# kianmcevoy/audio_analysis

Hardware: AMD Instinct MI355X
Metric: IRs/sec full report (STFT+RT60bands+zplane), 48 kHz 10 s IR (higher is better)
Workload: dtype f64; 1 GPU; metrics-only full report on 256 mono synthetic IRs per GPU per step, 10 s @ 48 kHz (SURVEY.md 8d generator), H2D included: every step uploads its batch from pinned host memory (float32, 492 MB) on a copy stream under the previous step's kernels; 4 distinct batches rotate; batch_per_gpu=256, parallelism=file-sharded dp1, gather=final

## Files before the change

### audio_analysis_amd/_lib.py

```python
from __future__ import annotations

import ctypes as C
from pathlib import Path

_LIB_PATH = Path(__file__).resolve().parent / "csrc" / "libira.so"
_lib = None
ABI_VERSION = 15

c_f32p = C.c_void_p
c_i64p = C.c_void_p
c_i32p = C.c_void_p
c_f64p = C.c_void_p
vp = C.c_void_p
i32 = C.c_int32
f64 = C.c_double
f32 = C.c_float

PROTOTYPES = {
    "ira_abi_version": (i32, []),
    "ira_error_string": (C.c_char_p, [i32]),
    "ira_peak_index": (i32, [vp, vp, vp, i32, C.c_int64, vp, vp, vp]),
    "ira_edc_db": (i32, [vp, vp, vp, i32, C.c_int64, f64, f64, vp, vp, vp, vp, vp]),
    "ira_curve_fits": (i32, [vp, vp, vp, i32, i32, f32, f32, vp, C.POINTER(f64), i32, i32, C.POINTER(f64), i32, i32,
                             f64, f64, vp, vp, vp]),
    "ira_edc_box_smooth": (i32, [vp, vp, vp, i32, C.c_int64, i32, f64, vp, vp]),
    "ira_edc_fits": (i32, [vp, vp, vp, i32, C.c_int64, f64, f64, f32, f32, C.POINTER(f64), i32, i32, C.POINTER(f64), i32,
                           vp, vp, vp, vp, vp, vp, vp, vp, vp, vp]),
    "ira_stft_mag_db": (i32, [vp, vp, vp, i32, i32, i32, i32, vp, vp, i32, f64, vp, vp, vp, vp, vp]),
    "ira_stft_logbin": (i32, [vp, vp, vp, i32, i32, i32, i32, vp, vp, i32, f64, i32, vp, vp, i32, vp, vp, vp]),
    "ira_stft_mag_db_tf": (i32, [vp, vp, vp, i32, i32, i32, i32, vp, vp, i32, f64, vp, vp, vp, vp, vp]),
    "ira_tail_energy": (i32, [vp, vp, vp, vp, i32, i32, vp, vp]),
    "ira_stft_logbin_tail": (i32, [vp, vp, vp, i32, i32, i32, i32, vp, vp, i32, f64, i32, vp, vp, i32, vp, vp, vp, vp, vp,
                                   vp]),
    "ira_stft_mag_db_tf_tail": (i32, [vp, vp, vp, i32, i32, i32, i32, vp, vp, i32, f64, vp, vp, vp, vp, vp, vp, vp, vp]),
    "ira_fft_split": (i32, [i32, vp, vp]),
    "ira_bluestein_filter": (i32, [vp, i32, i32, vp, vp, vp, vp, vp]),
    "ira_rfft_any": (i32, [vp, vp, vp, i32, i32, i32, vp, vp, vp, vp, vp, vp, vp, vp, vp, vp, vp, vp, i32, vp, vp, vp, vp,
                           vp, i32, vp]),
    "ira_band_irfft": (i32, [vp, vp, vp, i32, vp, vp, i32, vp, vp, vp, vp, vp, vp, vp, vp, vp, vp, vp]),
    "ira_spectrum_mag_phase": (i32, [vp, vp, vp, i32, i32, f64, vp, vp, vp, vp, vp, vp]),
    "ira_phase_unwrap": (i32, [vp, vp, vp, i32, i32, i32, vp, vp, vp, vp]),
    "ira_log_smooth_db": (i32, [vp, vp, vp, vp, vp, vp, vp, vp, vp, i32, i32, i32, i32, vp]),
    "ira_group_delay": (i32, [vp, vp, vp, i32, i32, vp, f64, vp, i32, vp, vp]),
    "ira_fft_smooth_split": (i32, [i32, vp, vp]),
    "ira_rfft_smooth": (i32, [vp, vp, i32, i32, i32, vp, vp, vp, vp, vp, vp, vp, vp, vp, vp, vp, vp, vp, vp, i32, vp]),
    "ira_band_irfft_smooth": (i32, [vp, vp, i32, i32, vp, vp, vp, vp, vp, vp, vp, vp, vp, vp, i32, vp, vp, vp]),
    "ira_band_tile_layout": (i32, [i32, i32, C.POINTER(i32), C.POINTER(i32)]),
    "ira_wav_probe": (i32, [C.c_char_p, vp, vp, vp, vp]),
    "ira_wav_read_pcm16": (i32, [C.c_char_p, C.c_int64, C.c_int64, i32, vp]),
    "ira_wav_probe_batch": (i32, [vp, i32, i32, vp, vp, vp, vp, vp]),
    "ira_wav_read_pcm16_batch": (i32, [vp, vp, vp, vp, vp, vp, i32, i32, vp]),
    "ira_pcm16_to_channels": (i32, [vp, C.c_int64, i32, i32, vp, vp]),
    "ira_pcm16_to_channels_jobs": (i32, [vp, vp, vp, vp, vp, vp, i32, C.c_int64, vp, vp]),
    "ira_band_mask_values": (i32, [C.POINTER(f64), f64, C.c_int64, vp, vp]),
    "ira_host_pull": (i32, [vp, C.c_int64, i32, vp, i32, vp]),
    "ira_deconv_divide": (i32, [vp, vp, vp, vp, vp, i32, i32, f64, vp, vp]),
    "ira_deconv_finish": (i32, [vp, vp, vp, vp, i32, i32, i32, i32, i32, f64, vp, vp, vp]),
    "ira_order_stats": (i32, [vp, vp, vp, i32, vp, i32, vp, vp]),
    "ira_diffusion": (i32, [vp, vp, vp, i32, i32, i32, i32, i32, f64, f64, vp, vp, vp, vp]),
    "ira_diffusion_stereo": (i32, [vp, vp, vp, vp, i32, i32, i32, i32, i32, vp, vp, vp, vp]),
    "ira_spectrum_stats": (i32, [vp, vp, vp, i32, vp, f64, f64, f64, vp, vp]),
    "ira_spectrum_finish": (i32, [vp, vp, vp, i32, f64, vp, vp, vp, i32, i32, vp, vp, vp, vp, f64, f64, f64, vp, vp]),
    "ira_waterfall_rel": (i32, [vp, vp, vp, i32, i32, i32, i32, f64, vp, vp, vp]),
    "ira_logbin_aggregate": (i32, [vp, vp, vp, i32, i32, i32, vp, vp, i32, vp, vp, i32, vp]),
    "ira_ar_partial_doubles": (C.c_int64, [i32, i32]),
    "ira_ar_gram": (i32, [vp, vp, vp, vp, vp, i32, i32, i32, vp, i32, vp]),
    "ira_ar_solve": (i32, [vp, vp, i32, i32, i32, f64, vp, vp, vp, i32, vp]),
# ... 87 lines not shown
```

### audio_analysis_amd/build.py

```python
from __future__ import annotations

import os
import shutil
import subprocess
import sys
from concurrent.futures import ThreadPoolExecutor
from pathlib import Path

CSRC = Path(__file__).resolve().parent / "csrc"
LIB = CSRC / "libira.so"
ARCH = "gfx950"

SOURCES = {
    "ira_api.hip": [],
    "ira_edc.hip": ["-ffp-contract=off"],
    "ira_stft.hip": ["-fno-slp-vectorize"],
    "ira_stft2.hip": ["-fno-slp-vectorize"],
    "ira_stft3.hip": ["-fno-slp-vectorize"],
    "ira_stft4.hip": [],
    "ira_tailenergy.hip": [],
    "ira_fftlong.hip": [],
    "ira_fftsmooth.hip": [],
    "ira_spectrum.hip": ["-ffp-contract=off"],
    "ira_modal.hip": ["-ffp-contract=off"],
    "ira_ar.hip": [],
    "ira_roots.hip": [],
    "ira_ingest.hip": ["-ffp-contract=off"],
    "ira_deconv.hip": ["-ffp-contract=off"],
    "ira_diffusion.hip": ["-ffp-contract=off"],
    "ira_energy.hip": ["-ffp-contract=off"],
    "ira_xcorr.hip": ["-ffp-contract=off"],
    "ira_lundeby.hip": ["-ffp-contract=off"],
    "ira_multislope.hip": ["-ffp-contract=off"],
    "ira_mtf.hip": [],
    "ira_harmonics.hip": ["-ffp-contract=off"],
    "ira_echo.hip": ["-ffp-contract=off"],
    "ira_echodensity.hip": ["-ffp-contract=off"],
    "ira_reflections.hip": ["-ffp-contract=off"],
    "ira_xspec.hip": [],
}
COMMON = ["-O3", "-std=c++17", "-fPIC", f"--offload-arch={ARCH}", "-Wall", "-Wno-unused-function"]


def _hipcc() -> str:
    exe = shutil.which("hipcc") or "/opt/rocm/bin/hipcc"
    if not Path(exe).exists():
        raise RuntimeError("hipcc not found; libira cannot be built")
    return exe


def _stale(obj: Path, deps) -> bool:
    if not obj.exists():
        return True
# ... 63 lines not shown
```

### audio_analysis_amd/csrc/ira_stft.h

```cpp
#pragma once
#include "ira_common.h"

int32_t ira_stft3_launch(const float* x, const int64_t* off, const int32_t* nframes, int32_t nseg, int32_t max_frames,
                         int32_t hop, const void* window, const void* tw, double floor_db, float* out,
                         const int64_t* out_off, const int32_t* frame_sel, const int64_t* sel_off, hipStream_t st);

int32_t ira_stft6_launch(const float* x, const int64_t* off, const int32_t* nframes, int32_t nseg, int32_t max_frames,
                         int32_t hop, const void* window, const void* tw, double floor_db, float* out,
                         const int64_t* out_off, const int32_t* frame_sel, const int64_t* sel_off, const double* tail,
                         const int64_t* tail_off, hipStream_t st);

int32_t ira_stft2_launch(const float* x, const int64_t* off, const int32_t* nframes, int32_t nseg, int32_t max_frames,
                         int32_t n_fft, int32_t hop, const void* window, const void* tw, int32_t precision,
                         double floor_db, float* out, const int64_t* out_off, const int32_t* frame_sel,
                         const int64_t* sel_off, hipStream_t st);

int32_t ira_stft5_launch(const float* x, const int64_t* off, const int32_t* nframes, int32_t nseg, int32_t max_frames,
                         int32_t hop, const void* window, const void* tw, double floor_db, float* out,
                         const int64_t* out_off, const int32_t* frame_sel, const int64_t* sel_off, int32_t lb_nbins,
                         int32_t lb_kbase, const int32_t* lb_first, const int32_t* lb_count, const double* tail,
                         const int64_t* tail_off, void* consts, hipStream_t st);
```

### audio_analysis_amd/csrc/ira_stft.hip

```cpp
#include <cmath>
#include <cstdlib>

#include "ira_fft_lds.h"
#include "ira_stft.h"

namespace {

using ira::cplx;

constexpr int STFT_THREADS = 256;

template <typename T>
__device__ __forceinline__ float mag_to_db(T re, T im, T floor_lin);

template <>
__device__ __forceinline__ float mag_to_db<float>(float re, float im, float floor_lin) {
  const float a = sqrtf(re * re + im * im);
  const float m = (a != a) ? a : fmaxf(a, floor_lin);
  return 20.0f * log10f(m);
}
template <>
__device__ __forceinline__ float mag_to_db<double>(double re, double im, double floor_lin) {
  const double a = hypot(re, im);
  const double m = (a != a) ? a : fmax(a, floor_lin);
// ... 91 lines not shown
                                   int32_t nseg, int32_t max_frames, int32_t n_fft, int32_t hop,
                                   const void* window_dev, const void* twiddle_dev, int32_t precision,
                                   double floor_db, float* out_dev, const int64_t* out_off_dev,
                                   const int32_t* frame_sel_dev, const int64_t* sel_off_dev, void* stream) {
  IRA_CHECK_PTR(x_dev); IRA_CHECK_PTR(off_dev); IRA_CHECK_PTR(nframes_dev); IRA_CHECK_PTR(window_dev);
  IRA_CHECK_PTR(twiddle_dev); IRA_CHECK_PTR(out_dev); IRA_CHECK_PTR(out_off_dev);
  if (frame_sel_dev != nullptr && sel_off_dev == nullptr) return IRA_E_NULL;
  if (nseg < 0 || max_frames < 0 || hop <= 0) return IRA_E_SIZE;
  if (nseg == 0 || max_frames == 0) return IRA_OK;
  if (n_fft < 64 || n_fft > 16384 || (n_fft & (n_fft - 1)) != 0) return IRA_E_SIZE;
  int log2n = 0;
  while ((1 << log2n) < n_fft) ++log2n;
  hipStream_t st = (hipStream_t)stream;
  if (precision != 32 && precision != 64) return IRA_E_UNSUPPORTED;
  if (precision == 32 && n_fft == 4096)
    return ira_stft3_launch(x_dev, off_dev, nframes_dev, nseg, max_frames, hop, window_dev, twiddle_dev, floor_db,
                            out_dev, out_off_dev, frame_sel_dev, sel_off_dev, st);
  if (n_fft == 8192 || (precision == 64 && n_fft == 4096))
    return ira_stft2_launch(x_dev, off_dev, nframes_dev, nseg, max_frames, n_fft, hop, window_dev, twiddle_dev,
                            precision, floor_db, out_dev, out_off_dev, frame_sel_dev, sel_off_dev, st);
  if (precision == 32)
    return launch_stft<float>(x_dev, off_dev, nframes_dev, nseg, max_frames, log2n, hop, window_dev, twiddle_dev,
                              floor_db, out_dev, out_off_dev, frame_sel_dev, sel_off_dev, st);
  return launch_stft<double>(x_dev, off_dev, nframes_dev, nseg, max_frames, log2n, hop, window_dev, twiddle_dev,
                             floor_db, out_dev, out_off_dev, frame_sel_dev, sel_off_dev, st);
}

namespace {

int32_t stft_mag_db_tf(const float* x_dev, const int64_t* off_dev, const int32_t* nframes_dev, int32_t nseg,
                       int32_t max_frames, int32_t n_fft, int32_t hop, const void* window_dev, const void* twiddle_dev,
                       int32_t precision, double floor_db, float* out_dev, const int64_t* out_off_dev,
                       const int32_t* frame_sel_dev, const int64_t* sel_off_dev, const double* tail_dev,
                       const int64_t* tail_off_dev, void* consts_dev, void* stream) {
  IRA_CHECK_PTR(x_dev); IRA_CHECK_PTR(off_dev); IRA_CHECK_PTR(nframes_dev); IRA_CHECK_PTR(window_dev);
  IRA_CHECK_PTR(twiddle_dev); IRA_CHECK_PTR(out_dev); IRA_CHECK_PTR(out_off_dev);
  if (frame_sel_dev != nullptr && sel_off_dev == nullptr) return IRA_E_NULL;
  if (nseg < 0 || max_frames < 0 || hop <= 0) return IRA_E_SIZE;
  if (nseg == 0 || max_frames == 0) return IRA_OK;
  if (nseg > 65535) return IRA_E_SIZE;
  hipStream_t st = (hipStream_t)stream;
  if (precision == 32 && n_fft == 4096)
    return ira_stft6_launch(x_dev, off_dev, nframes_dev, nseg, max_frames, hop, window_dev, twiddle_dev, floor_db,
                            out_dev, out_off_dev, frame_sel_dev, sel_off_dev, tail_dev, tail_off_dev, st);
  if (precision == 64 && n_fft == 8192)
    return ira_stft5_launch(x_dev, off_dev, nframes_dev, nseg, max_frames, hop, window_dev, twiddle_dev, floor_db,
                            out_dev, out_off_dev, frame_sel_dev, sel_off_dev, 0, 0, nullptr, nullptr, tail_dev,
                            tail_off_dev, consts_dev, st);
  return IRA_E_UNSUPPORTED;
}

int32_t stft_logbin(const float* x_dev, const int64_t* off_dev, const int32_t* nframes_dev, int32_t nseg,
                    int32_t max_frames, int32_t n_fft, int32_t hop, const void* window_dev, const void* twiddle_dev,
                    int32_t precision, double floor_db, int32_t k_base, const int32_t* first_dev,
                    const int32_t* count_dev, int32_t nbins, float* curves_dev, const int64_t* curves_off_dev,
                    const double* tail_dev, const int64_t* tail_off_dev, void* consts_dev, void* stream) {
  IRA_CHECK_PTR(x_dev); IRA_CHECK_PTR(off_dev); IRA_CHECK_PTR(nframes_dev); IRA_CHECK_PTR(window_dev);
  IRA_CHECK_PTR(twiddle_dev); IRA_CHECK_PTR(first_dev); IRA_CHECK_PTR(count_dev); IRA_CHECK_PTR(curves_dev);
  IRA_CHECK_PTR(curves_off_dev);
  if (nseg < 0 || max_frames < 0 || hop <= 0 || nbins <= 0 || k_base < 0) return IRA_E_SIZE;
  if (nseg == 0 || max_frames == 0) return IRA_OK;
  if (nseg > 65535) return IRA_E_SIZE;
  if (precision != 64 || n_fft != 8192) return IRA_E_UNSUPPORTED;
  return ira_stft5_launch(x_dev, off_dev, nframes_dev, nseg, max_frames, hop, window_dev, twiddle_dev, floor_db,
                          curves_dev, curves_off_dev, nullptr, nullptr, nbins, k_base, first_dev, count_dev, tail_dev,
                          tail_off_dev, consts_dev, (hipStream_t)stream);
}

}

extern "C" int32_t ira_stft_mag_db_tf(const float* x_dev, const int64_t* off_dev, const int32_t* nframes_dev,
                                      int32_t nseg, int32_t max_frames, int32_t n_fft, int32_t hop,
                                      const void* window_dev, const void* twiddle_dev, int32_t precision,
                                      double floor_db, float* out_dev, const int64_t* out_off_dev,
                                      const int32_t* frame_sel_dev, const int64_t* sel_off_dev, void* stream) {
  return stft_mag_db_tf(x_dev, off_dev, nframes_dev, nseg, max_frames, n_fft, hop, window_dev, twiddle_dev, precision,
                        floor_db, out_dev, out_off_dev, frame_sel_dev, sel_off_dev, nullptr, nullptr, nullptr, stream);
}

extern "C" int32_t ira_stft_mag_db_tf_tail(const float* x_dev, const int64_t* off_dev, const int32_t* nframes_dev,
                                           int32_t nseg, int32_t max_frames, int32_t n_fft, int32_t hop,
                                           const void* window_dev, const void* twiddle_dev, int32_t precision,
                                           double floor_db, float* out_dev, const int64_t* out_off_dev,
                                           const int32_t* frame_sel_dev, const int64_t* sel_off_dev,
                                           const double* tail_dev, const int64_t* tail_off_dev, void* consts_dev,
                                           void* stream) {
  return stft_mag_db_tf(x_dev, off_dev, nframes_dev, nseg, max_frames, n_fft, hop, window_dev, twiddle_dev, precision,
                        floor_db, out_dev, out_off_dev, frame_sel_dev, sel_off_dev, tail_dev, tail_off_dev, consts_dev,
                        stream);
}

extern "C" int32_t ira_stft_logbin(const float* x_dev, const int64_t* off_dev, const int32_t* nframes_dev,
                                   int32_t nseg, int32_t max_frames, int32_t n_fft, int32_t hop,
                                   const void* window_dev, const void* twiddle_dev, int32_t precision, double floor_db,
                                   int32_t k_base, const int32_t* first_dev, const int32_t* count_dev, int32_t nbins,
                                   float* curves_dev, const int64_t* curves_off_dev, void* stream) {
  return stft_logbin(x_dev, off_dev, nframes_dev, nseg, max_frames, n_fft, hop, window_dev, twiddle_dev, precision,
                     floor_db, k_base, first_dev, count_dev, nbins, curves_dev, curves_off_dev, nullptr, nullptr, nullptr,
                     stream);
}

extern "C" int32_t ira_stft_logbin_tail(const float* x_dev, const int64_t* off_dev, const int32_t* nframes_dev,
                                        int32_t nseg, int32_t max_frames, int32_t n_fft, int32_t hop,
                                        const void* window_dev, const void* twiddle_dev, int32_t precision,
                                        double floor_db, int32_t k_base, const int32_t* first_dev,
                                        const int32_t* count_dev, int32_t nbins, float* curves_dev,
                                        const int64_t* curves_off_dev, const double* tail_dev,
                                        const int64_t* tail_off_dev, void* consts_dev, void* stream) {
  return stft_logbin(x_dev, off_dev, nframes_dev, nseg, max_frames, n_fft, hop, window_dev, twiddle_dev, precision,
                     floor_db, k_base, first_dev, count_dev, nbins, curves_dev, curves_off_dev, tail_dev, tail_off_dev,
                     consts_dev, stream);
}
```

### audio_analysis_amd/csrc/ira_stft4.hip

```cpp
#include <cmath>
#include <cstdlib>

#include "ira_fft_reg.h"
#include "ira_log.h"
#include "ira_stft.h"

namespace {

using ira::brev_bits;
using ira::cplx;
using ira::dft_dif;
using ira::powers16;

typedef cplx<double> cdd;

constexpr int M4 = 4096, F4 = M4 + 1, TL4 = 128;
constexpr int ROW4 = 129;
constexpr int E2N4 = 256;
constexpr int EXC4 = 16 * ROW4;
static_assert(EXC4 >= 8 * E2N4 && EXC4 * 2 >= M4, "exchange buffer too small");

__device__ __forceinline__ float db_of4(double re, double im, double floor_pow, float floor_db,
                                        const ira::LogTabEntry* tab) {
  const double p = fma(re, re, im * im);
// ... 56 lines not shown
  for (int o = 32; o > 0; o >>= 1) {
    const unsigned long long other = __shfl_xor(wb, o, 64);
    wb = other > wb ? other : wb;
  }
  if ((q & 63) == 0) wmax[q >> 6] = wb;
  __syncthreads();
  unsigned long long wm = wmax[0];
#pragma unroll
  for (int i = 1; i < TL5 / 64; ++i) wm = wmax[i] > wm ? wmax[i] : wm;
  return ira::uniform(__longlong_as_double((long long)wm));
}

__global__ __launch_bounds__(TL5) void stft5_consts_kernel(const double* __restrict__ window, float floor_db, int lb_nbins,
                                                           const int32_t* __restrict__ lb_count, Stft5Consts* __restrict__ cst) {
  __shared__ unsigned long long wmax[TL5 / 64];
  __shared__ ira::LogTabEntry ltab[ira::LOGTAB_N];
  const int q = threadIdx.x;
  ira::build_log_table(ltab, q);
  const double wmax2 = window_max_sq5(window, q, wmax);
  if (q == 0) cst->wmax2 = wmax2;
  const double floor_lin32 = ira::uniform(exp10((double)floor_db * 0.05));
  for (int bb = q; bb < lb_nbins; bb += TL5) {
    const int c = lb_count[bb];
    cst->row[bb] = c > 0 ? logbin_mean_db<true>(nullptr, floor_lin32, c, ltab) : __uint_as_float(0x7fc00000u);
  }
}

__global__ __launch_bounds__(TL5) __attribute__((amdgpu_waves_per_eu(4, 4))) void stft5_kernel(
    const float* __restrict__ x, const int64_t* __restrict__ off, const int32_t* __restrict__ nframes, int hop,
    const double* __restrict__ window, const cdd* __restrict__ tw, double floor_lin, float floor_db,
    float* __restrict__ out, const int64_t* __restrict__ out_off, const int32_t* __restrict__ frame_sel,
    const int64_t* __restrict__ sel_off, int lb_nbins, int lb_kbase, const int32_t* __restrict__ lb_first,
    const int32_t* __restrict__ lb_count, int kfr, int ablate, const double* __restrict__ tail,
    const int64_t* __restrict__ tail_off, const Stft5Consts* __restrict__ cst) {
  __shared__ __attribute__((aligned(16))) cdd ex[EXC4];
  __shared__ double wave_energy[2][TL5 / 64];
  __shared__ double chunk_energy[TL5 / 64];
  __shared__ unsigned long long chunk_wmax[TL5 / 64];
  __shared__ float quiet_val[TL5];
  __shared__ ira::LogTabEntry ltab[ira::LOGTAB_N];
  __shared__ int lb_range[2];
  __shared__ int frame_bad;
  unsigned bx, by;
  ira::xcd_remap(bx, by);
  const int seg = (int)by;
  const int col0 = (int)bx * kfr;
  const int T_out = ira::uniform(nframes[seg]);
  if (col0 >= T_out) return;
  const int col1 = T_out - col0 < kfr ? T_out : col0 + kfr;
  int q = threadIdx.x;
  float* os = out + ira::uniform(out_off[seg]);
  const double floor_pow = floor_lin * floor_lin;

  const bool use_tail = tail != nullptr && frame_sel == nullptr && !IRA_ABL(ablate & (256 | 512));
  if (use_tail) {
    const int64_t j = ((int64_t)col0 * hop) / IRA_TAIL_BLOCK;
    const double S = ira::uniform(tail[ira::uniform(tail_off[seg]) + j]);
    const double wmax2 = ira::uniform(cst->wmax2);
    if (S * (4.0 * (2 * M4)) * wmax2 <= floor_pow) {
      const int nfr = col1 - col0;
      if (lb_nbins <= 0) {
        float* fo = os + (int64_t)col0 * F4;
        for (int i = q; i < nfr * F4; i += TL5) fo[i] = floor_db;
      } else {
        for (int bb = q; bb < lb_nbins; bb += TL5) {
          const float val = cst->row[bb];
          float* o = os + (int64_t)bb * T_out + col0;
          for (int jf = 0; jf < nfr; ++jf) o[jf] = val;
        }
      }
      return;
    }
  }

  double* exd = reinterpret_cast<double*>(ex);
  ira::build_log_table(ltab, q);
  if (q < 2) lb_range[q] = q == 0 ? F4 : 0;

  const float* xs = x + ira::uniform(off[seg]);
// ... 237 lines not shown
        if (!need_a && !need_b) continue;
        const cdd e = {0.5 * (zkr[i] + zpr[i]), 0.5 * (zki[i] - zpi[i])};
        const cdd d = {0.5 * (zkr[i] - zpr[i]), 0.5 * (zki[i] + zpi[i])};
        const cdd o = {d.im, -d.re};
        const cdd wk = ira::cmul(wlane, wuni[i]);
        const cdd pp = ira::cmul(wk, o);
        if (IRA_ABL(ablate & 4)) {
          if (need_a) exd[k] = e.re + pp.re;
          if (need_b) exd[M4 - k] = e.im - pp.im;
          continue;
        }
        if (need_a) exd[k] = lin_of4(e.re + pp.re, e.im + pp.im, floor_pow, floor_db, floor_lin32, ltab);
        if (need_b) exd[M4 - k] = lin_of4(e.re - pp.re, e.im - pp.im, floor_pow, floor_db, floor_lin32, ltab);
      }
      if (q == 0 && M4 / 2 >= k_lo && M4 / 2 < k_hi) exd[M4 / 2] = lin_of4(midr, midi, floor_pow, floor_db, floor_lin32, ltab);
    }
    __syncthreads();
    for (int bb = q; bb < lb_nbins; bb += TL5) {
      const int c = lb_count[bb];
      float val = qnan32;
      if (c > 0) val = logbin_mean_db<false>(exd + lb_kbase + lb_first[bb], 0.0, c, ltab);
      os[(int64_t)bb * T_out + col] = (bad_frame && c > 0) ? qnan32 : val;
    }
    __syncthreads();
  }
}

}

int32_t ira_stft5_launch(const float* x, const int64_t* off, const int32_t* nframes, int32_t nseg, int32_t max_frames,
                         int32_t hop, const void* window, const void* tw, double floor_db, float* out,
                         const int64_t* out_off, const int32_t* frame_sel, const int64_t* sel_off, int32_t lb_nbins,
                         int32_t lb_kbase, const int32_t* lb_first, const int32_t* lb_count, const double* tail,
                         const int64_t* tail_off, void* consts, hipStream_t st) {
  const double floor_lin = std::pow(10.0, floor_db / 20.0);
  int kfr = ira_tune_int("IRA_STFT5_K", KF5);
  if (kfr < 1) kfr = 1;
  if (frame_sel != nullptr) tail = nullptr;
  if (tail != nullptr) {
    if (tail_off == nullptr || consts == nullptr) return IRA_E_NULL;
    stft5_consts_kernel<<<1, TL5, 0, st>>>(static_cast<const double*>(window), (float)floor_db, lb_nbins > 0 ? lb_nbins : 0,
                                           lb_count, static_cast<Stft5Consts*>(consts));
    IRA_TRY_HIP(hipGetLastError());
  }
  dim3 grid((max_frames + kfr - 1) / kfr, nseg);
  stft5_kernel<<<grid, TL5, (size_t)ira_tune_int("IRA_STFT5_LDS_PAD", 0), st>>>(x, off, nframes, hop, static_cast<const double*>(window),
                                     static_cast<const cdd*>(tw), floor_lin, (float)floor_db, out, out_off, frame_sel,
                                     sel_off, lb_nbins, lb_kbase, lb_first, lb_count, kfr, ira_tune_int("IRA_STFT5_ABLATE", 0),
                                     tail, tail_off, static_cast<const Stft5Consts*>(consts));
  IRA_RETURN_LAUNCH();
}
```

### audio_analysis_amd/engine.py

```python
from __future__ import annotations

import ctypes
import math
import os
from contextlib import contextmanager
from dataclasses import dataclass, fields
from typing import Dict, List, Optional, Sequence, Tuple

import numpy as np

from . import _lib
from ._lib import IraError, check
from .engine_plan import (SMOOTH, Switches, conv_size, exclusive_cumsum, pair_bands, plan_band_irfft,
                          plan_rfft)

FIT_DOUBLES = 8
EDC_SCRATCH_DOUBLES = 4096
EDC_TILE = 4096


def _ptr(t) -> int:
    return 0 if t is None else int(t.data_ptr())


# ... 980 lines not shown
        if not np.array_equal(np.asarray(tail["start"]), np.asarray(seg_off, dtype=np.int64)):
            raise ValueError("the suffix-energy table was made for other segment starts")
        last = np.asarray(seg_off, dtype=np.int64) + (cols.astype(np.int64) - 1) * int(hop) + int(n_fft)
        if np.any((cols > 0) & (last > np.asarray(tail["end"]))):
            raise ValueError("a frame reads past the end the suffix-energy table was made for")
        return tail["tab"], tail["off_dev"]

    def stft_mag_db(self, x_dev, seg_off: np.ndarray, nframes: np.ndarray, n_fft: int, hop: int, use_hann: bool,
                    floor_db: float, precision: int = 32, frame_sel: Optional[List[np.ndarray]] = None,
                    frame_major: bool = False, tail=None):
        t = self.torch
        n = int(seg_off.size)
        f = n_fft // 2 + 1
        if self.stft_generic_needed(n_fft):
            return self._stft_generic(x_dev, seg_off, nframes, int(n_fft), int(hop), use_hann, floor_db, frame_sel,
                                      frame_major)
        if frame_sel is not None:
            cols = np.array([int(s.size) for s in frame_sel], dtype=np.int32)
            sel_off = exclusive_cumsum(cols)
            if cols.sum():
                sel, sel_off_dev = self.job_tables(np.concatenate(frame_sel).astype(np.int32), sel_off)
            else:
                sel, sel_off_dev = self.empty(1, t.int32), self.to_dev(sel_off)
        else:
            cols = np.ascontiguousarray(nframes, dtype=np.int32)
            sel = None
            sel_off_dev = None
        sizes = cols.astype(np.int64) * f
        out_off = exclusive_cumsum(sizes)
        out = self.empty(int(sizes.sum()), t.float32)
        d_off, d_cols, d_ooff = self.job_tables(seg_off, cols, out_off)
        use_tail = tail is not None and frame_major and frame_sel is None and self.stft_tail_ok(n_fft, precision) and n > 0
        name = "ira_stft_mag_db_tf_tail" if use_tail else "ira_stft_mag_db_tf" if frame_major else "ira_stft_mag_db"
        extra = ()
        if use_tail:
            d_tab, d_toff = self._tail_args(tail, seg_off, cols, n_fft, hop)
            consts = self.empty(1, t.float64)
            extra = (_ptr(d_tab), _ptr(d_toff), _ptr(consts))
        with self.tagged(f"[f{precision},n{n_fft}{',sel' if frame_sel is not None else ''}]"):
            check(getattr(self.lib, name)(
                _ptr(x_dev), _ptr(d_off), _ptr(d_cols), n, int(cols.max()) if n else 0, int(n_fft), int(hop),
                _ptr(self.window(n_fft, use_hann, precision)), _ptr(self.twiddle(n_fft, precision)), int(precision),
                float(floor_db), _ptr(out), _ptr(d_ooff), _ptr(sel), _ptr(sel_off_dev), *extra, self.stream), name)
        return out, out_off, cols

    def stft_logbin(self, x_dev, seg_off: np.ndarray, nframes: np.ndarray, n_fft: int, hop: int, use_hann: bool,
                    floor_db: float, k_base: int, first: np.ndarray, count: np.ndarray, tail=None):
        t = self.torch
        n = int(seg_off.size)
        nbins = int(first.size)
        cols = np.ascontiguousarray(nframes, dtype=np.int32)
        sizes = cols.astype(np.int64) * nbins
        out_off = exclusive_cumsum(sizes)
        out = self.empty(int(sizes.sum()), t.float32)
        d_off, d_cols, d_ooff, d_f, d_c = self.job_tables(seg_off, cols, out_off, first.astype(np.int32),
                                                           count.astype(np.int32))
        name, extra = "ira_stft_logbin", ()
        if tail is not None and n > 0:
            d_tab, d_toff = self._tail_args(tail, seg_off, cols, n_fft, hop)
            name = "ira_stft_logbin_tail"
            consts = self.empty(1 + (nbins + 1) // 2, t.float64)
            extra = (_ptr(d_tab), _ptr(d_toff), _ptr(consts))
        with self.tagged(f"[f64,n{n_fft}]"):
            check(getattr(self.lib, name)(_ptr(x_dev), _ptr(d_off), _ptr(d_cols), n, int(cols.max()) if n else 0,
                                          int(n_fft), int(hop), _ptr(self.window(n_fft, use_hann, 64)),
                                          _ptr(self.twiddle(n_fft, 64)), 64, float(floor_db), int(k_base), _ptr(d_f),
                                          _ptr(d_c), nbins, _ptr(out), _ptr(d_ooff), *extra, self.stream), name)
        return out, out_off

    @staticmethod
    def stft_generic_needed(n_fft: int) -> bool:
        n = int(n_fft)
        return n < 64 or n > 16384 or (n & (n - 1)) != 0

    def _stft_generic(self, x_dev, seg_off, nframes, n_fft: int, hop: int, use_hann: bool, floor_db: float, frame_sel,
                      frame_major: bool):
        t = self.torch
        n = int(seg_off.size)
        f = n_fft // 2 + 1
        if frame_sel is not None:
            frames = [np.asarray(s_, dtype=np.int64) for s_ in frame_sel]
        else:
            frames = [np.arange(int(c), dtype=np.int64) for c in nframes]
        cols = np.array([fr.size for fr in frames], dtype=np.int32)
        sizes = cols.astype(np.int64) * f
        out_off = exclusive_cumsum(sizes)
        total_frames = int(cols.sum())
        if total_frames == 0:
            return self.empty(1, t.float32), out_off, cols
        xoff = np.concatenate([int(seg_off[i]) + fr * int(hop) for i, fr in enumerate(frames)])
        lengths = np.full(total_frames, n_fft, dtype=np.int32)
        spec, spec_off = self.rfft_any(x_dev, xoff, lengths, bool(use_hann))
        mag, _ = self.spectrum_mag_phase(spec, spec_off, lengths, float(floor_db), want_phase=False)
        if frame_major:
            return mag, out_off, cols
# ... 502 lines not shown
```

### include/ira.h

```cpp
#ifndef IRA_H_
#define IRA_H_

#include <stdint.h>

#ifdef __cplusplus
extern "C" {
#endif

#define IRA_OK 0
#define IRA_E_NULL (-1)
#define IRA_E_SIZE (-2)
#define IRA_E_UNSUPPORTED (-3)
#define IRA_E_IO (-4)
#define IRA_E_FORMAT (-5)
#define IRA_E_HIP_BASE (-1000)

#define IRA_ABI_VERSION 15

int32_t ira_abi_version(void);
const char* ira_error_string(int32_t code);

int32_t ira_peak_index(const float* x_dev, const int64_t* off_dev, const int64_t* len_dev,
                       int32_t nseg, int64_t max_len, int64_t* peak_dev, float* peak_abs_dev, void* stream);

// ... 27 lines not shown
                        const void* window_dev, const void* twiddle_dev, int32_t precision,
                        double floor_db, float* out_dev, const int64_t* out_off_dev,
                        const int32_t* frame_sel_dev, const int64_t* sel_off_dev, void* stream);

int32_t ira_stft_mag_db_tf(const float* x_dev, const int64_t* off_dev, const int32_t* nframes_dev,
                           int32_t nseg, int32_t max_frames, int32_t n_fft, int32_t hop,
                           const void* window_dev, const void* twiddle_dev, int32_t precision,
                           double floor_db, float* out_dev, const int64_t* out_off_dev,
                           const int32_t* frame_sel_dev, const int64_t* sel_off_dev, void* stream);

int32_t ira_stft_logbin(const float* x_dev, const int64_t* off_dev, const int32_t* nframes_dev, int32_t nseg,
                        int32_t max_frames, int32_t n_fft, int32_t hop, const void* window_dev,
                        const void* twiddle_dev, int32_t precision, double floor_db, int32_t k_base,
                        const int32_t* first_dev, const int32_t* count_dev, int32_t nbins, float* curves_dev,
                        const int64_t* curves_off_dev, void* stream);

#define IRA_TAIL_BLOCK 512
int32_t ira_tail_energy(const float* x_dev, const int64_t* start_dev, const int64_t* end_dev,
                        const int64_t* tab_off_dev, int32_t nseg, int32_t max_nblk, double* tab_dev, void* stream);

#define IRA_STFT_CONSTS_DOUBLES(nbins) (1 + ((nbins) + 1) / 2)
int32_t ira_stft_logbin_tail(const float* x_dev, const int64_t* off_dev, const int32_t* nframes_dev, int32_t nseg,
                             int32_t max_frames, int32_t n_fft, int32_t hop, const void* window_dev,
                             const void* twiddle_dev, int32_t precision, double floor_db, int32_t k_base,
                             const int32_t* first_dev, const int32_t* count_dev, int32_t nbins, float* curves_dev,
                             const int64_t* curves_off_dev, const double* tail_dev, const int64_t* tail_off_dev,
                             void* consts_dev, void* stream);
int32_t ira_stft_mag_db_tf_tail(const float* x_dev, const int64_t* off_dev, const int32_t* nframes_dev,
                                int32_t nseg, int32_t max_frames, int32_t n_fft, int32_t hop,
                                const void* window_dev, const void* twiddle_dev, int32_t precision,
                                double floor_db, float* out_dev, const int64_t* out_off_dev,
                                const int32_t* frame_sel_dev, const int64_t* sel_off_dev, const double* tail_dev,
                                const int64_t* tail_off_dev, void* consts_dev, void* stream);


int32_t ira_fft_split(int32_t m, int32_t* n1, int32_t* n2);

int32_t ira_bluestein_filter(const int32_t* L_dev, int32_t nfilt, int32_t m, const void* t1_dev,
                             const void* t2_dev, const void* tf_dev, double* bfilt_dev, void* stream);

int32_t ira_rfft_any(const float* x_dev, const int64_t* xoff_dev, const int32_t* L_dev, int32_t nb,
                     int32_t use_hann, int32_t m, const void* t1_dev, const void* t2_dev,
                     const void* tf_dev, const double* bfilt_dev, const int32_t* bidx_dev,
                     double* work_dev, double* spec_out_dev, const int64_t* spec_off_dev,
                     const int64_t* x2off_dev, const int64_t* spec_off2_dev, double* zpair_dev,
                     const int64_t* zpair_off_dev, int32_t max_len, const int32_t* data_len_dev,
                     const int32_t* win_len_dev, const int32_t* data_len2_dev, const int32_t* win_len2_dev,
                     const int32_t* interleave_dev, int32_t keep_packed, void* stream);

#define IRA_BAND_DOUBLES 8
int32_t ira_band_irfft(const double* spec_dev, const int64_t* spec_off_dev, const int32_t* L_dev,
                       int32_t nb, const double* band_params_dev, const double* freq_val_dev,
                       int32_t m, const void* t1_dev, const void* t2_dev, const void* tf_dev,
                       const double* bfilt_dev, const int32_t* bidx_dev, double* work_dev, float* y_dev,
                       const int64_t* y1_off_dev, const int64_t* y2_off_dev,
                       const int64_t* spec_off2_dev, void* stream);

int32_t ira_spectrum_mag_phase(const double* spec_dev, const int64_t* spec_off_dev, const int32_t* L_dev,
                               int32_t nb, int32_t max_len, double floor_db, float* mag_db_dev,
                               const int64_t* mag_off_dev, double* phase_dev,
                               const int64_t* phase_off_dev, const int32_t* packed_dev, void* stream);

int32_t ira_phase_unwrap(const double* phase_dev, const int64_t* phase_off_dev, const int32_t* L_dev,
                         int32_t nb, int32_t do_unwrap, int32_t to_degrees, float* out_dev,
                         const int64_t* out_off_dev, double* out64_dev, void* stream);

// ... 247 lines not shown
```

Baseline: 17580 IRs/s.

## Cut STFT frames below the noise floor using tail-energy bounds and compact grid

Adds a cut kernel that uses per-block tail-energy tables to find, for each segment, the first frame chunk after which every frame is certified to sit at the dB floor. A prefix scan turns these cuts into a compacted work list, so the f64 STFT kernel only launches blocks for chunks that need computing, and a vectorized fill kernel writes the floor value (or per-bin floor row) into the skipped region. This removes FFT work on silent IR tails at the cost of two small extra launches plus a fill pass, and it relies on the certification bound being conservative.

Measured after the change: 17520 IRs/s. About the same (-0.3%).

```diff
diff --git a/audio_analysis_amd/_lib.py b/audio_analysis_amd/_lib.py
--- a/audio_analysis_amd/_lib.py
+++ b/audio_analysis_amd/_lib.py
@@ -33,6 +33,9 @@
     "ira_stft_logbin_tail": (i32, [vp, vp, vp, i32, i32, i32, i32, vp, vp, i32, f64, i32, vp, vp, i32, vp, vp, vp, vp, vp,
                                    vp]),
     "ira_stft_mag_db_tf_tail": (i32, [vp, vp, vp, i32, i32, i32, i32, vp, vp, i32, f64, vp, vp, vp, vp, vp, vp, vp, vp]),
+    "ira_stft_logbin_cut": (i32, [vp, vp, vp, i32, i32, i32, i32, vp, vp, i32, f64, i32, vp, vp, i32, vp, vp, vp, vp, vp,
+                                  vp, vp]),
+    "ira_stft_mag_db_tf_cut": (i32, [vp, vp, vp, i32, i32, i32, i32, vp, vp, i32, f64, vp, vp, vp, vp, vp, vp, vp]),
     "ira_fft_split": (i32, [i32, vp, vp]),
     "ira_bluestein_filter": (i32, [vp, i32, i32, vp, vp, vp, vp, vp]),
     "ira_rfft_any": (i32, [vp, vp, vp, i32, i32, i32, vp, vp, vp, vp, vp, vp, vp, vp, vp, vp, vp, vp, i32, vp, vp, vp, vp,
diff --git a/audio_analysis_amd/build.py b/audio_analysis_amd/build.py
--- a/audio_analysis_amd/build.py
+++ b/audio_analysis_amd/build.py
@@ -19,6 +19,7 @@
     "ira_stft3.hip": ["-fno-slp-vectorize"],
     "ira_stft4.hip": [],
     "ira_tailenergy.hip": [],
+    "ira_stftcut.hip": [],
     "ira_fftlong.hip": [],
     "ira_fftsmooth.hip": [],
     "ira_spectrum.hip": ["-ffp-contract=off"],
diff --git a/audio_analysis_amd/csrc/ira_stft.h b/audio_analysis_amd/csrc/ira_stft.h
--- a/audio_analysis_amd/csrc/ira_stft.h
+++ b/audio_analysis_amd/csrc/ira_stft.h
@@ -19,4 +19,10 @@
                          int32_t hop, const void* window, const void* tw, double floor_db, float* out,
                          const int64_t* out_off, const int32_t* frame_sel, const int64_t* sel_off, int32_t lb_nbins,
                          int32_t lb_kbase, const int32_t* lb_first, const int32_t* lb_count, const double* tail,
-                         const int64_t* tail_off, void* consts, hipStream_t st);
+                         const int64_t* tail_off, void* consts, int32_t* work, hipStream_t st);
+
+int32_t ira_stft_cut_launch(const int32_t* nframes, int32_t nseg, int32_t hop, int32_t unit, const void* consts,
+                            double floor_pow, const double* tail, const int64_t* tail_off, int32_t* work, hipStream_t st);
+int32_t ira_stft_fill_launch(const int32_t* nframes, int32_t nseg, int32_t max_frames, const int64_t* out_off, float* out,
+                             int32_t unit, int32_t rowlen, float val, const float* row, int32_t nruns, const int32_t* work,
+                             hipStream_t st);
diff --git a/audio_analysis_amd/csrc/ira_stft.hip b/audio_analysis_amd/csrc/ira_stft.hip
--- a/audio_analysis_amd/csrc/ira_stft.hip
+++ b/audio_analysis_amd/csrc/ira_stft.hip
@@ -147,7 +147,7 @@
                        int32_t max_frames, int32_t n_fft, int32_t hop, const void* window_dev, const void* twiddle_dev,
                        int32_t precision, double floor_db, float* out_dev, const int64_t* out_off_dev,
                        const int32_t* frame_sel_dev, const int64_t* sel_off_dev, const double* tail_dev,
-                       const int64_t* tail_off_dev, void* consts_dev, void* stream) {
+                       const int64_t* tail_off_dev, void* consts_dev, int32_t* work_dev, void* stream) {
   IRA_CHECK_PTR(x_dev); IRA_CHECK_PTR(off_dev); IRA_CHECK_PTR(nframes_dev); IRA_CHECK_PTR(window_dev);
   IRA_CHECK_PTR(twiddle_dev); IRA_CHECK_PTR(out_dev); IRA_CHECK_PTR(out_off_dev);
   if (frame_sel_dev != nullptr && sel_off_dev == nullptr) return IRA_E_NULL;
@@ -155,13 +155,14 @@
   if (nseg == 0 || max_frames == 0) return IRA_OK;
   if (nseg > 65535) return IRA_E_SIZE;
   hipStream_t st = (hipStream_t)stream;
+  if (work_dev != nullptr && precision != 64) return IRA_E_UNSUPPORTED;
   if (precision == 32 && n_fft == 4096)
     return ira_stft6_launch(x_dev, off_dev, nframes_dev, nseg, max_frames, hop, window_dev, twiddle_dev, floor_db,
                             out_dev, out_off_dev, frame_sel_dev, sel_off_dev, tail_dev, tail_off_dev, st);
   if (precision == 64 && n_fft == 8192)
     return ira_stft5_launch(x_dev, off_dev, nframes_dev, nseg, max_frames, hop, window_dev, twiddle_dev, floor_db,
                             out_dev, out_off_dev, frame_sel_dev, sel_off_dev, 0, 0, nullptr, nullptr, tail_dev,
-                            tail_off_dev, consts_dev, st);
+                            tail_off_dev, consts_dev, work_dev, st);
   return IRA_E_UNSUPPORTED;
 }
 
@@ -169,7 +170,8 @@
                     int32_t max_frames, int32_t n_fft, int32_t hop, const void* window_dev, const void* twiddle_dev,
                     int32_t precision, double floor_db, int32_t k_base, const int32_t* first_dev,
                     const int32_t* count_dev, int32_t nbins, float* curves_dev, const int64_t* curves_off_dev,
-                    const double* tail_dev, const int64_t* tail_off_dev, void* consts_dev, void* stream) {
+                    const double* tail_dev, const int64_t* tail_off_dev, void* consts_dev, int32_t* work_dev,
+                    void* stream) {
   IRA_CHECK_PTR(x_dev); IRA_CHECK_PTR(off_dev); IRA_CHECK_PTR(nframes_dev); IRA_CHECK_PTR(window_dev);
   IRA_CHECK_PTR(twiddle_dev); IRA_CHECK_PTR(first_dev); IRA_CHECK_PTR(count_dev); IRA_CHECK_PTR(curves_dev);
   IRA_CHECK_PTR(curves_off_dev);
@@ -179,7 +181,7 @@
   if (precision != 64 || n_fft != 8192) return IRA_E_UNSUPPORTED;
   return ira_stft5_launch(x_dev, off_dev, nframes_dev, nseg, max_frames, hop, window_dev, twiddle_dev, floor_db,
                           curves_dev, curves_off_dev, nullptr, nullptr, nbins, k_base, first_dev, count_dev, tail_dev,
-                          tail_off_dev, consts_dev, (hipStream_t)stream);
+                          tail_off_dev, consts_dev, work_dev, (hipStream_t)stream);
 }
 
 }
@@ -190,7 +192,7 @@
                                       double floor_db, float* out_dev, const int64_t* out_off_dev,
                                       const int32_t* frame_sel_dev, const int64_t* sel_off_dev, void* stream) {
   return stft_mag_db_tf(x_dev, off_dev, nframes_dev, nseg, max_frames, n_fft, hop, window_dev, twiddle_dev, precision,
-                        floor_db, out_dev, out_off_dev, frame_sel_dev, sel_off_dev, nullptr, nullptr, nullptr, stream);
+                        floor_db, out_dev, out_off_dev, frame_sel_dev, sel_off_dev, nullptr, nullptr, nullptr, nullptr, stream);
 }
 
 extern "C" int32_t ira_stft_mag_db_tf_tail(const float* x_dev, const int64_t* off_dev, const int32_t* nframes_dev,
@@ -202,6 +204,18 @@
                                            void* stream) {
   return stft_mag_db_tf(x_dev, off_dev, nframes_dev, nseg, max_frames, n_fft, hop, window_dev, twiddle_dev, precision,
                         floor_db, out_dev, out_off_dev, frame_sel_dev, sel_off_dev, tail_dev, tail_off_dev, consts_dev,
+                        nullptr, stream);
+}
+
+extern "C" int32_t ira_stft_mag_db_tf_cut(const float* x_dev, const int64_t* off_dev, const int32_t* nframes_dev,
+                                          int32_t nseg, int32_t max_frames, int32_t n_fft, int32_t hop,
+                                          const void* window_dev, const void* twiddle_dev, int32_t precision,
+                                          double floor_db, float* out_dev, const int64_t* out_off_dev,
+                                          const double* tail_dev, const int64_t* tail_off_dev, void* consts_dev,
+                                          int32_t* work_dev, void* stream) {
+  IRA_CHECK_PTR(tail_dev); IRA_CHECK_PTR(tail_off_dev); IRA_CHECK_PTR(work_dev);
+  return stft_mag_db_tf(x_dev, off_dev, nframes_dev, nseg, max_frames, n_fft, hop, window_dev, twiddle_dev, precision,
+                        floor_db, out_dev, out_off_dev, nullptr, nullptr, tail_dev, tail_off_dev, consts_dev, work_dev,
                         stream);
 }
 
@@ -212,7 +226,7 @@
                                    float* curves_dev, const int64_t* curves_off_dev, void* stream) {
   return stft_logbin(x_dev, off_dev, nframes_dev, nseg, max_frames, n_fft, hop, window_dev, twiddle_dev, precision,
                      floor_db, k_base, first_dev, count_dev, nbins, curves_dev, curves_off_dev, nullptr, nullptr, nullptr,
-                     stream);
+                     nullptr, stream);
 }
 
 extern "C" int32_t ira_stft_logbin_tail(const float* x_dev, const int64_t* off_dev, const int32_t* nframes_dev,
@@ -224,5 +238,17 @@
                                         const int64_t* tail_off_dev, void* consts_dev, void* stream) {
   return stft_logbin(x_dev, off_dev, nframes_dev, nseg, max_frames, n_fft, hop, window_dev, twiddle_dev, precision,
                      floor_db, k_base, first_dev, count_dev, nbins, curves_dev, curves_off_dev, tail_dev, tail_off_dev,
-                     consts_dev, stream);
-}
+                     consts_dev, nullptr, stream);
+}
+
+extern "C" int32_t ira_stft_logbin_cut(const float* x_dev, const int64_t* off_dev, const int32_t* nframes_dev, int32_t nseg,
+                                       int32_t max_frames, int32_t n_fft, int32_t hop, const void* window_dev,
+                                       const void* twiddle_dev, int32_t precision, double floor_db, int32_t k_base,
+                                       const int32_t* first_dev, const int32_t* count_dev, int32_t nbins, float* curves_dev,
+                                       const int64_t* curves_off_dev, const double* tail_dev, const int64_t* tail_off_dev,
+                                       void* consts_dev, int32_t* work_dev, void* stream) {
+  IRA_CHECK_PTR(tail_dev); IRA_CHECK_PTR(tail_off_dev); IRA_CHECK_PTR(work_dev);
+  return stft_logbin(x_dev, off_dev, nframes_dev, nseg, max_frames, n_fft, hop, window_dev, twiddle_dev, precision,
+                     floor_db, k_base, first_dev, count_dev, nbins, curves_dev, curves_off_dev, tail_dev, tail_off_dev,
+                     consts_dev, work_dev, stream);
+}
diff --git a/audio_analysis_amd/csrc/ira_stft4.hip b/audio_analysis_amd/csrc/ira_stft4.hip
--- a/audio_analysis_amd/csrc/ira_stft4.hip
+++ b/audio_analysis_amd/csrc/ira_stft4.hip
@@ -112,7 +112,8 @@
     float* __restrict__ out, const int64_t* __restrict__ out_off, const int32_t* __restrict__ frame_sel,
     const int64_t* __restrict__ sel_off, int lb_nbins, int lb_kbase, const int32_t* __restrict__ lb_first,
     const int32_t* __restrict__ lb_count, int kfr, int ablate, const double* __restrict__ tail,
-    const int64_t* __restrict__ tail_off, const Stft5Consts* __restrict__ cst) {
+    const int64_t* __restrict__ tail_off, const Stft5Consts* __restrict__ cst, int nseg,
+    const int32_t* __restrict__ work) {
   __shared__ __attribute__((aligned(16))) cdd ex[EXC4];
   __shared__ double wave_energy[2][TL5 / 64];
   __shared__ double chunk_energy[TL5 / 64];
@@ -121,10 +122,26 @@
   __shared__ ira::LogTabEntry ltab[ira::LOGTAB_N];
   __shared__ int lb_range[2];
   __shared__ int frame_bad;
-  unsigned bx, by;
-  ira::xcd_remap(bx, by);
-  const int seg = (int)by;
-  const int col0 = (int)bx * kfr;
+  int seg, col0;
+  if (work != nullptr) {
+    const unsigned xcd = blockIdx.x & 7u, k = blockIdx.x >> 3;
+    const unsigned total = (unsigned)ira::uniform(work[nseg]);
+    const unsigned per = (total + 7u) >> 3;
+    const unsigned i = xcd * per + k;
+    if (k >= per || i >= total) return;
+    int lo = 0, hi = nseg;
+    while (hi - lo > 1) {
+      const int mid = (lo + hi) >> 1;
+      if ((unsigned)ira::uniform(work[mid]) <= i) lo = mid; else hi = mid;
+    }
+    seg = lo;
+    col0 = (int)(i - (unsigned)ira::uniform(work[lo])) * kfr;
+  } else {
+    unsigned bx, by;
+    ira::xcd_remap(bx, by);
+    seg = (int)by;
+    col0 = (int)bx * kfr;
+  }
   const int T_out = ira::uniform(nframes[seg]);
   if (col0 >= T_out) return;
   const int col1 = T_out - col0 < kfr ? T_out : col0 + kfr;
@@ -428,11 +445,12 @@
                          int32_t hop, const void* window, const void* tw, double floor_db, float* out,
                          const int64_t* out_off, const int32_t* frame_sel, const int64_t* sel_off, int32_t lb_nbins,
                          int32_t lb_kbase, const int32_t* lb_first, const int32_t* lb_count, const double* tail,
-                         const int64_t* tail_off, void* consts, hipStream_t st) {
+                         const int64_t* tail_off, void* consts, int32_t* work, hipStream_t st) {
   const double floor_lin = std::pow(10.0, floor_db / 20.0);
   int kfr = ira_tune_int("IRA_STFT5_K", KF5);
   if (kfr < 1) kfr = 1;
   if (frame_sel != nullptr) tail = nullptr;
+  if (tail == nullptr || ira_tune_int("IRA_STFT5_ABLATE", 0) != 0) work = nullptr;
   if (tail != nullptr) {
     if (tail_off == nullptr || consts == nullptr) return IRA_E_NULL;
     stft5_consts_kernel<<<1, TL5, 0, st>>>(static_cast<const double*>(window), (float)floor_db, lb_nbins > 0 ? lb_nbins : 0,
@@ -440,9 +458,20 @@
     IRA_TRY_HIP(hipGetLastError());
   }
   dim3 grid((max_frames + kfr - 1) / kfr, nseg);
+  if (work != nullptr) {
+    const int32_t rc = ira_stft_cut_launch(nframes, nseg, hop, kfr, consts, floor_lin * floor_lin, tail, tail_off, work, st);
+    if (rc != IRA_OK) return rc;
+    const uint64_t chunks = (uint64_t)grid.x * (uint64_t)nseg;
+    if (chunks > 0x7ffffff8ull) return IRA_E_SIZE;
+    grid = dim3((unsigned)((chunks + 7) & ~(uint64_t)7));
+  }
   stft5_kernel<<<grid, TL5, (size_t)ira_tune_int("IRA_STFT5_LDS_PAD", 0), st>>>(x, off, nframes, hop, static_cast<const double*>(window),
                                      static_cast<const cdd*>(tw), floor_lin, (float)floor_db, out, out_off, frame_sel,
                                      sel_off, lb_nbins, lb_kbase, lb_first, lb_count, kfr, ira_tune_int("IRA_STFT5_ABLATE", 0),
-                                     tail, tail_off, static_cast<const Stft5Consts*>(consts));
-  IRA_RETURN_LAUNCH();
-}
+                                     tail, tail_off, static_cast<const Stft5Consts*>(consts), nseg, work);
+  IRA_TRY_HIP(hipGetLastError());
+  if (work == nullptr) return IRA_OK;
+  const Stft5Consts* cst = static_cast<const Stft5Consts*>(consts);
+  return ira_stft_fill_launch(nframes, nseg, max_frames, out_off, out, kfr, lb_nbins > 0 ? 0 : F4, (float)floor_db, cst->row,
+                              lb_nbins > 0 ? lb_nbins : 1, work, st);
+}
diff --git a/audio_analysis_amd/csrc/ira_stftcut.hip b/audio_analysis_amd/csrc/ira_stftcut.hip
--- /dev/null
+++ b/audio_analysis_amd/csrc/ira_stftcut.hip
@@ -0,0 +1,127 @@
+#include "ira_reduce.h"
+#include "ira_stft.h"
+
+namespace {
+
+constexpr int CUT_THREADS = 256;
+constexpr int FILL_Q = 16;
+
+__device__ __forceinline__ bool cert5(const double* __restrict__ S, int64_t frame, int hop, double wmax2, double floor_pow) {
+  const int64_t j = (frame * hop) / IRA_TAIL_BLOCK;
+  return S[j] * (4.0 * (2 * 4096)) * wmax2 <= floor_pow;
+}
+
+__global__ __launch_bounds__(CUT_THREADS) void stft_cut_kernel(const int32_t* __restrict__ nframes, int hop, int unit,
+                                                               const double* __restrict__ wmax2_dev, double floor_pow,
+                                                               const double* __restrict__ tail,
+                                                               const int64_t* __restrict__ tail_off, int nseg,
+                                                               int32_t* __restrict__ work) {
+  __shared__ int cut_s;
+  const int seg = blockIdx.x, tid = threadIdx.x;
+  const int T = ira::uniform(nframes[seg]);
+  const double* S = tail + ira::uniform(tail_off[seg]);
+  const double wmax2 = ira::uniform(*wmax2_dev);
+  if (tid == 0) cut_s = 0;
+  __syncthreads();
+  const int nunits = (T + unit - 1) / unit;
+  int cut = 0;
+  for (int u = tid; u < nunits; u += CUT_THREADS)
+    if (!cert5(S, (int64_t)u * unit, hop, wmax2, floor_pow)) cut = u + 1;
+  cut = ira::wave_max_int(cut);
+  if ((tid & 63) == 0 && cut > 0) atomicMax(&cut_s, cut);
+  __syncthreads();
+  if (tid == 0) work[nseg + 1 + seg] = cut_s;
+}
+
+__global__ __launch_bounds__(256) void stft_first_kernel(int nseg, int32_t* __restrict__ work) {
+  __shared__ int wtot[4];
+  __shared__ int carry_s;
+  const int tid = threadIdx.x, lane = tid & 63, wave = tid >> 6;
+  const int32_t* cut = work + nseg + 1;
+  if (tid == 0) carry_s = 0;
+  __syncthreads();
+  for (int s0 = 0; s0 < nseg; s0 += 256) {
+    const int s = s0 + tid;
+    int excl;
+    const int incl = ira::wave_prefix(s < nseg ? cut[s] : 0, lane, excl);
+    if (lane == 63) wtot[wave] = incl;
+    __syncthreads();
+    int base = carry_s;
+    for (int w = 0; w < wave; ++w) base += wtot[w];
+    if (s < nseg) work[s] = base + excl;
+    __syncthreads();
+    if (tid == 255) carry_s = base + incl;
+    __syncthreads();
+  }
+  if (tid == 0) work[nseg] = carry_s;
+}
+
+__global__ __launch_bounds__(256) void stft_fill_kernel(const int32_t* __restrict__ nframes, const int64_t* __restrict__ out_off,
+                                                        float* __restrict__ out, int unit, int rowlen, float val,
+                                                        const float* __restrict__ row, int nruns, int nseg,
+                                                        const int32_t* __restrict__ work) {
+  const int seg = blockIdx.z, lane = threadIdx.x & 63, nw = blockDim.x >> 6;
+  const int wave = __builtin_amdgcn_readfirstlane((int)(threadIdx.x >> 6));
+  const int T = ira::uniform(nframes[seg]);
+  const int64_t c64 = (int64_t)ira::uniform(work[nseg + 1 + seg]) * unit;
+  if (c64 >= T) return;
+  const int c = (int)c64;
+  float* p;
+  int64_t n, piece;
+  float v = val;
+  if (rowlen > 0) {
+    p = out + ira::uniform(out_off[seg]) + (int64_t)c * rowlen;
+    n = (int64_t)(T - c) * rowlen;
+    piece = (int64_t)blockIdx.x * nw + wave;
+  } else {
+    const int r = (int)blockIdx.y * nw + wave;
+    if (r >= nruns) return;
+    p = out + ira::uniform(out_off[seg]) + (int64_t)r * T + c;
+    n = T - c;
+    piece = blockIdx.x;
+    v = ira::uniform(row[r]);
+  }
+  int64_t head = (int64_t)((16u - (unsigned)((uintptr_t)p & 15u)) & 15u) >> 2;
+  if (head > n) head = n;
+  const int64_t nq = (n - head) >> 2;
+  const int64_t q0 = piece * (FILL_Q * IRA_WAVE);
+  if (q0 >= nq && piece != 0) return;
+  typedef float f4 __attribute__((ext_vector_type(4)));
+  f4* body = reinterpret_cast<f4*>(p + head);
+  const f4 v4 = {v, v, v, v};
+#pragma unroll
+  for (int u = 0; u < FILL_Q; ++u) {
+    const int64_t q = q0 + u * IRA_WAVE + lane;
+    if (q < nq) body[q] = v4;
+  }
+  if (piece == 0) {
+    if (lane < head) p[lane] = v;
+    const int64_t done = head + 4 * nq;
+    if (done + lane < n && lane < 3) p[done + lane] = v;
+  }
+}
+
+}
+
+int32_t ira_stft_cut_launch(const int32_t* nframes, int32_t nseg, int32_t hop, int32_t unit, const void* consts,
+                            double floor_pow, const double* tail, const int64_t* tail_off, int32_t* work, hipStream_t st) {
+  stft_cut_kernel<<<nseg, CUT_THREADS, 0, st>>>(nframes, hop, unit, static_cast<const double*>(consts), floor_pow, tail,
+                                                tail_off, nseg, work);
+  IRA_TRY_HIP(hipGetLastError());
+  stft_first_kernel<<<1, 256, 0, st>>>(nseg, work);
+  IRA_RETURN_LAUNCH();
+}
+
+int32_t ira_stft_fill_launch(const int32_t* nframes, int32_t nseg, int32_t max_frames, const int64_t* out_off, float* out,
+                             int32_t unit, int32_t rowlen, float val, const float* row, int32_t nruns, const int32_t* work,
+                             hipStream_t st) {
+  const int64_t run_quads = ((int64_t)max_frames * (rowlen > 0 ? rowlen : 1)) / 4 + 1;
+  const int64_t pieces = ira::ceil_div(run_quads, FILL_Q * IRA_WAVE);
+  const int nw = 4;
+  const int64_t gx = rowlen > 0 ? ira::ceil_div(pieces, nw) : pieces;
+  const int64_t gy = rowlen > 0 ? 1 : ira::ceil_div(nruns, nw);
+  if (gx > 0x7fffffffll || gy > 65535 || nseg > 65535) return IRA_E_SIZE;
+  stft_fill_kernel<<<dim3((unsigned)gx, (unsigned)gy, (unsigned)nseg), nw * IRA_WAVE, 0, st>>>(
+      nframes, out_off, out, unit, rowlen, val, row, nruns, nseg, work);
+  IRA_RETURN_LAUNCH();
+}
diff --git a/audio_analysis_amd/engine.py b/audio_analysis_amd/engine.py
--- a/audio_analysis_amd/engine.py
+++ b/audio_analysis_amd/engine.py
@@ -1036,16 +1036,20 @@
         d_off, d_cols, d_ooff = self.job_tables(seg_off, cols, out_off)
         use_tail = tail is not None and frame_major and frame_sel is None and self.stft_tail_ok(n_fft, precision) and n > 0
         name = "ira_stft_mag_db_tf_tail" if use_tail else "ira_stft_mag_db_tf" if frame_major else "ira_stft_mag_db"
-        extra = ()
+        extra = (_ptr(sel), _ptr(sel_off_dev))
         if use_tail:
             d_tab, d_toff = self._tail_args(tail, seg_off, cols, n_fft, hop)
             consts = self.empty(1, t.float64)
-            extra = (_ptr(d_tab), _ptr(d_toff), _ptr(consts))
+            extra += (_ptr(d_tab), _ptr(d_toff), _ptr(consts))
+            if int(precision) == 64:
+                name = "ira_stft_mag_db_tf_cut"
+                work = self.empty(2 * (n + 1), t.int32)
+                extra = (_ptr(d_tab), _ptr(d_toff), _ptr(consts), _ptr(work))
         with self.tagged(f"[f{precision},n{n_fft}{',sel' if frame_sel is not None else ''}]"):
             check(getattr(self.lib, name)(
                 _ptr(x_dev), _ptr(d_off), _ptr(d_cols), n, int(cols.max()) if n else 0, int(n_fft), int(hop),
                 _ptr(self.window(n_fft, use_hann, precision)), _ptr(self.twiddle(n_fft, precision)), int(precision),
-                float(floor_db), _ptr(out), _ptr(d_ooff), _ptr(sel), _ptr(sel_off_dev), *extra, self.stream), name)
+                float(floor_db), _ptr(out), _ptr(d_ooff), *extra, self.stream), name)
         return out, out_off, cols
 
     def stft_logbin(self, x_dev, seg_off: np.ndarray, nframes: np.ndarray, n_fft: int, hop: int, use_hann: bool,
@@ -1062,9 +1066,10 @@
         name, extra = "ira_stft_logbin", ()
         if tail is not None and n > 0:
             d_tab, d_toff = self._tail_args(tail, seg_off, cols, n_fft, hop)
-            name = "ira_stft_logbin_tail"
+            name = "ira_stft_logbin_cut"
             consts = self.empty(1 + (nbins + 1) // 2, t.float64)
-            extra = (_ptr(d_tab), _ptr(d_toff), _ptr(consts))
+            work = self.empty(2 * (n + 1), t.int32)
+            extra = (_ptr(d_tab), _ptr(d_toff), _ptr(consts), _ptr(work))
         with self.tagged(f"[f64,n{n_fft}]"):
             check(getattr(self.lib, name)(_ptr(x_dev), _ptr(d_off), _ptr(d_cols), n, int(cols.max()) if n else 0,
                                           int(n_fft), int(hop), _ptr(self.window(n_fft, use_hann, 64)),
diff --git a/include/ira.h b/include/ira.h
--- a/include/ira.h
+++ b/include/ira.h
@@ -83,6 +83,19 @@
                                 double floor_db, float* out_dev, const int64_t* out_off_dev,
                                 const int32_t* frame_sel_dev, const int64_t* sel_off_dev, const double* tail_dev,
                                 const int64_t* tail_off_dev, void* consts_dev, void* stream);
+
+#define IRA_STFT_WORK_INTS(nseg) (2 * ((nseg) + 1))
+int32_t ira_stft_logbin_cut(const float* x_dev, const int64_t* off_dev, const int32_t* nframes_dev, int32_t nseg,
+                            int32_t max_frames, int32_t n_fft, int32_t hop, const void* window_dev,
+                            const void* twiddle_dev, int32_t precision, double floor_db, int32_t k_base,
+                            const int32_t* first_dev, const int32_t* count_dev, int32_t nbins, float* curves_dev,
+                            const int64_t* curves_off_dev, const double* tail_dev, const int64_t* tail_off_dev,
+                            void* consts_dev, int32_t* work_dev, void* stream);
+int32_t ira_stft_mag_db_tf_cut(const float* x_dev, const int64_t* off_dev, const int32_t* nframes_dev,
+                               int32_t nseg, int32_t max_frames, int32_t n_fft, int32_t hop,
+                               const void* window_dev, const void* twiddle_dev, int32_t precision,
+                               double floor_db, float* out_dev, const int64_t* out_off_dev, const double* tail_dev,
+                               const int64_t* tail_off_dev, void* consts_dev, int32_t* work_dev, void* stream);
 
 
 int32_t ira_fft_split(int32_t m, int32_t* n1, int32_t* n2);
```
